# RQLuo/CDLNet-video

Hardware: AMD Instinct MI355X
Metric: Mpix/s denoised (fwd+bwd) at K=30,M=64,P=7 (higher is better)
Workload: dtype f32 (split-bf16 x3 MFMA, fp32 accumulate, fp32 storage)

## Files before the change

### cdlnet-video_amd/csrc/cdl_common.h

```cpp
#pragma once
#include <hip/hip_runtime.h>
#include "../../include/cdlnet_hip.h"

#define CDL_LAUNCH_CHECK()                                   \
    do {                                                     \
        hipError_t e_ = hipGetLastError();                   \
        if (e_ != hipSuccess) return -(int)e_;               \
    } while (0)

__device__ __forceinline__ float cdl_shrink(float u, float t)
{
    float m = fabsf(u) - t;
    m = m > 0.0f ? m : (m != m ? m : 0.0f);
    const float s = u > 0.0f ? 1.0f : (u < 0.0f ? -1.0f : (u != u ? u : 0.0f));
    return s * m;
}

__device__ __forceinline__ float cdl_sgn(float x) { return x > 0.0f ? 1.0f : (x < 0.0f ? -1.0f : 0.0f); }

struct cdl_prox1 {
    float s, ls, a, tg, m, z;
};

__device__ __forceinline__ cdl_prox1 cdl_prox_csr1(float u, float zp, float lam, float gam)
// ... 51 lines not shown

__host__ __device__ __forceinline__ int cdl_floordiv(int a, int b)
{
    int q = a / b;
    return (a % b != 0 && ((a < 0) != (b < 0))) ? q - 1 : q;
}

#ifdef CDL_ABLATE
#define CDL_DBG(flags, bit) (((flags) & (bit)) != 0)
#define CDL_DBG_FIELD(decl) decl
#define CDL_DBG_COMMA(x) , x
#else
#define CDL_DBG(flags, bit) (false)
#define CDL_DBG_FIELD(decl)
#define CDL_DBG_COMMA(x)
#endif

struct cdl_options {
    int mfma_analysis, mfma_synthesis, mfma_wgrad, mfma_dense;
    int no_tiled, no_pipelined_synthesis;
    int fused_snake;
    int fused_grid;
    int fused_da;
    int fusedg_bwd_prec;
    int fusedg_strip;
    int scalar_assemble;
    int fused_debug, dense_debug;
};
const cdl_options &cdl_opts();
bool cdl_exact_fp32();
int cdl_current_device();
int cdl_cu_count();
int cdl_ensure_dynamic_lds(const void *kernel, int bytes);

static inline bool cdl_geom_ok(const cdl_geom *g)
{
    if (!g) return false;
    if (g->N <= 0 || g->C <= 0 || g->M <= 0) return false;
    if (g->D <= 0 || g->H <= 0 || g->W <= 0) return false;
    if (g->Pd <= 0 || g->Ph <= 0 || g->Pw <= 0) return false;
    if (g->sd <= 0 || g->sh <= 0 || g->sw <= 0) return false;
    if (g->pd < 0 || g->ph < 0 || g->pw < 0) return false;
    if (g->D % g->sd || g->H % g->sh || g->W % g->sw) return false;
    return true;
}

// ... 47 lines not shown
```

### cdlnet-video_amd/csrc/cdl_fused2d.hip

```cpp
#include <atomic>
#include <cstdlib>
#include <type_traits>
#include <mutex>
#include <utility>
#include <vector>

#include "cdl_common.h"

#ifdef CDL_F2D_WY4
#define CDL_WY 4
#define cdl_fused2d_assemble cdl_fused2d_assemble_wy4
#define cdl_fused2d_backward cdl_fused2d_backward_wy4
#define cdl_fused2d_code_bytes cdl_fused2d_code_bytes_wy4
#define cdl_fused2d_dtau_reduce cdl_fused2d_dtau_reduce_wy4
#define cdl_fused2d_forward cdl_fused2d_forward_wy4
#define cdl_fused2d_frag_bytes cdl_fused2d_frag_bytes_wy4
#define cdl_fused2d_iter_fwd cdl_fused2d_iter_fwd_wy4
#define cdl_fused2d_map_words cdl_fused2d_map_words_wy4
#define cdl_fused2d_patch_floats cdl_fused2d_patch_floats_wy4
#define cdl_fused2d_prep cdl_fused2d_prep_wy4
#define cdl_fused2d_stage_bwd cdl_fused2d_stage_bwd_wy4
#define cdl_fused2d_support_map cdl_fused2d_support_map_wy4
#define cdl_fused2d_supported cdl_fused2d_supported_wy4
#define cdl_fused2d_tiles cdl_fused2d_tiles_wy4
// ... 21 lines not shown
constexpr int RTW = TW + 2 * HALO, RTH = TH + 2 * HALO;
constexpr int RTC = RTW + 2;
constexpr int PITCH = WY == 2 ? 28 : 44;
constexpr int COPY = RTC * PITCH;
constexpr int LDS_RT = 2 * 4 * COPY * 2;
constexpr int SLAB = RTH * RTW;
constexpr int LDS_RSUM = 4 * SLAB * 4;
constexpr int LDS_W = 32 * 64 * 16;
constexpr int LDS_TAU = 64 * 4;
constexpr int LDS_TACC = NW * 64 * 4;
constexpr int LDS_STAGE = LDS_RT + LDS_RSUM + LDS_W + LDS_TAU + LDS_TACC;

constexpr int GW_TH = 16;
constexpr int GW_RTH = GW_TH + 2 * HALO;
constexpr int TROWS = GW_RTH + 1;
constexpr int TPITCH = 72;
constexpr int TCOPY = TROWS * TPITCH;
constexpr int WG_THIN_BYTES = 2 * 2 * 4 * TCOPY * 2;
constexpr int IMG_ELEMS = 32 * 32;

constexpr int LDS_DA_THIN = 2 * 4 * TCOPY * 2;
constexpr int LDS_DA = LDS_DA_THIN + NW * 2 * 2 * IMG_ELEMS * 2;

struct FusedParams {
    const float *r;
    const float *zin;
    unsigned *map;
    float *zout;
    const float *tau;
    float *dtau;
    const uint4 *frags;
    float *patches;
    float sgn;
    int do_synth;
    CDL_DBG_FIELD(int dbg;)
    int N, H, W, tilesX, tilesY;
    int rev;
    const float *r2;
    float *da_partial;
};

enum { MODE_FWD = 0, MODE_FIRST = 1, MODE_BWD = 2 };

__device__ __forceinline__ float embed7(const float *w, int P, int i, int j)
{
    const int off = (7 - P) / 2;
    const int ii = i - off, jj = j - off;
    if (i > 6 || j > 6 || ii < 0 || jj < 0 || ii >= P || jj >= P) return 0.0f;
    return w[ii * P + jj];
}

__device__ __forceinline__ void prep_one(const float *__restrict__ wA, const float *__restrict__ wB,
                                         uint4 *__restrict__ out, int MT, int P, int t)
{
    const int FA = MT * 4, FB = 4 * MT;
    if (t >= (FA + FB) * 64) return;
    const int lane = t & 63, f = t >> 6;
    const int row = lane & 31, h = lane >> 5;
    const int PP = P * P;
    float v[8];
    if (f < FA) {
        const int R = f / 4, ks = f % 4;
// ... 169 lines not shown
{
    return __builtin_bit_cast(float, __builtin_amdgcn_update_dpp(0, __builtin_bit_cast(int, v), 0x138, 0xf, 0xf, true));
}
__device__ __forceinline__ float upper_half_to_lower(float v)
{
    float lo = 0.0f;
    asm volatile("s_nop 1\n\tv_permlane32_swap_b32 %0, %1\n\ts_nop 1" : "+v"(v), "+v"(lo));
    return lo;
}
__device__ __forceinline__ float col2im_row(const float (&rv)[4], int h)
{
    const float r4 = upper_half_to_lower(rv[0]);
    const float r5 = upper_half_to_lower(rv[1]);
    const float r6 = upper_half_to_lower(rv[2]);
    const bool lo = h == 0;
    float s = lo ? r6 : 0.0f;
    s = wave_shr1(s) + (lo ? r5 : 0.0f);
    s = wave_shr1(s) + (lo ? r4 : 0.0f);
    s = wave_shr1(s) + (lo ? rv[3] : 0.0f);
    s = wave_shr1(s) + (lo ? rv[2] : 0.0f);
    s = wave_shr1(s) + (lo ? rv[1] : 0.0f);
    s = wave_shr1(s) + (lo ? rv[0] : 0.0f);
    return s;
}

template <int MT, int PREC, int MODE, int LIN, int LOUT, bool DA = false>
__global__ __launch_bounds__(NT) void k_stage(FusedParams p)
{
    static_assert(!DA || (MODE == MODE_BWD && TH == GW_TH), "dA_k rides in the reverse stage, on k_wgrad2d's 64 x 16 tiles");
    extern __shared__ __attribute__((aligned(16))) unsigned char smem[];
    __bf16 *rt = reinterpret_cast<__bf16 *>(smem);
    float *rsum_all = reinterpret_cast<float *>(smem + LDS_RT);
    const uint4 *wl = reinterpret_cast<const uint4 *>(smem + LDS_RT + LDS_RSUM);
    float *tau_s = reinterpret_cast<float *>(smem + LDS_RT + LDS_RSUM + LDS_W);
    float *tacc_s = tau_s + 64;
    __bf16 *thin2 = reinterpret_cast<__bf16 *>(smem + LDS_STAGE);
    __bf16 *imgs2 = reinterpret_cast<__bf16 *>(smem + LDS_STAGE + LDS_DA_THIN);

    constexpr int M = 32 * MT;
    constexpr int FA = MT * 4, FB = 4 * MT;
    constexpr int NFRAG = (PREC != 1 ? 2 : 1) * (FA + FB);
    constexpr int NSTG = (RTH * RTW + NT - 1) / NT;
    const int tid = threadIdx.x, lane = tid & 63, wid = tid >> 6;
    const int wxi = wid % WX, wyi = wid / WX;
    const int c = lane & 31, h = lane >> 5;
    const size_t HW = (size_t)p.H * p.W;
// ... 480 lines not shown
    stage_store();
    if constexpr (DA) stage2_store();
    }
    if constexpr (DA) {
        float *red = reinterpret_cast<float *>(smem);
        for (int w = 0; w < NW; ++w) {
            __syncthreads();
            if (wid == w) {
#pragma unroll
                for (int R = 0; R < MT; ++R)
#pragma unroll
                    for (int tt = 0; tt < 2; ++tt)
#pragma unroll
                        for (int v = 0; v < 16; ++v) {
                            const int ch = 32 * R + (v & 3) + 8 * (v >> 2) + 4 * h;
                            float *dstw = &red[ch * 64 + 32 * tt + c];
                            *dstw = (w == 0 ? 0.0f : *dstw) + dacc[R][tt][v];
                        }
            }
        }
        __syncthreads();
        float *dst = p.da_partial + (size_t)blockIdx.x * 2 * M * 64;
        for (int i = tid; i < M * 64; i += NT) dst[i] = red[i];
    }
}

__device__ __forceinline__ float patch_sum(const float *__restrict__ patches, int n, int Y, int X,
                                           int tilesX, int tilesY)
{
    const int tyc = Y / TH, txc = X / TW;
    const int ly = Y - tyc * TH, lx = X - txc * TW;
    const int hx = (lx < HALO && txc > 0) ? -1 : ((lx >= TW - HALO && txc + 1 < tilesX) ? 1 : 0);
    const int vy = (ly < HALO && tyc > 0) ? -1 : ((ly >= TH - HALO && tyc + 1 < tilesY) ? 1 : 0);
    const float *own = patches + (((size_t)n * tilesY + tyc) * tilesX + txc) * SLAB + (ly + HALO) * RTW + lx + HALO;
    const ptrdiff_t dx = (ptrdiff_t)hx * (SLAB - TW), dy = (ptrdiff_t)vy * ((ptrdiff_t)tilesX * SLAB - TH * RTW);
    float sum = 0.0f;
    if (vy < 0) {
        if (hx < 0) sum += own[dy + dx];
        sum += own[dy];
        if (hx > 0) sum += own[dy + dx];
    }
    if (hx < 0) sum += own[dx];
    sum += own[0];
    if (hx > 0) sum += own[dx];
    if (vy > 0) {
        if (hx < 0) sum += own[dy + dx];
// ... 95 lines not shown
    const size_t i = (size_t)blockIdx.x * blockDim.x + threadIdx.x;
    if (i >= (size_t)N * 2 * HW) return;
    const size_t pix = i % HW;
    const int h = (int)((i / HW) % 2), n = (int)(i / (2 * HW));
    unsigned ws = 0, wg = 0;
    for (int R = 0; R < M / 32; ++R)
        for (int v = 0; v < 16; ++v) {
            const int ch = 32 * R + 8 * (v >> 2) + 4 * h + (v & 3);
            const float zz = z[((size_t)n * M + ch) * HW + pix];
            ws |= (zz != 0.0f ? 1u : 0u) << (16 * R + v);
            wg |= (__builtin_bit_cast(unsigned, zz) >> 31) << (16 * R + v);
        }
    map[((size_t)n * 4 + 2 * h) * HW + pix] = ws;
    map[((size_t)n * 4 + 2 * h + 1) * HW + pix] = wg;
}

struct WgradParams {
    const float *X[2];
    const float *T[2];
    float *partial;
    int N, H, W, tilesX, tilesY, numTiles;
    int rev;
    int single;
};

template <int MT, int PREC, int LAY>
__global__ __launch_bounds__(512) void k_wgrad2d(WgradParams p)
{
    extern __shared__ __attribute__((aligned(16))) unsigned char dsm[];
    __bf16 *thin = reinterpret_cast<__bf16 *>(dsm);
    __bf16 *imgs = reinterpret_cast<__bf16 *>(dsm + WG_THIN_BYTES);
    constexpr int M = 32 * MT;
    const int tid = threadIdx.x, lane = tid & 63, wid = tid >> 6;
    const int op = wid >> 2, wq = wid & 3;
    const int wxi = wq & 1, wyi = wq >> 1;
    const int c = lane & 31, h = lane >> 5;
    const size_t HW = (size_t)p.H * p.W;
    __bf16 *wimg = imgs + (size_t)wid * (MT * 2) * IMG_ELEMS;
    f32x16 acc[MT][2];
#pragma unroll
    for (int R = 0; R < MT; ++R)
#pragma unroll
        for (int tt = 0; tt < 2; ++tt)
#pragma unroll
            for (int v = 0; v < 16; ++v) acc[R][tt][v] = 0.0f;

    for (int i = tid; i < WG_THIN_BYTES / 16; i += 512) reinterpret_cast<uint4 *>(dsm)[i] = make_uint4(0, 0, 0, 0);

    const bool present = p.X[op] != nullptr;
    const int nsteps = p.single ? (p.numTiles + 1) / 2 : p.numTiles;
    for (int t0 = blockIdx.x; t0 < nsteps; t0 += gridDim.x) {
        const int t = p.single ? 2 * t0 + op : t0;
        const bool active = present && t < p.numTiles;
        int bid = p.rev ? p.numTiles - 1 - t : t;
        const int txi = bid % p.tilesX; bid /= p.tilesX;
        const int tyi = bid % p.tilesY;
        const int n = active ? bid / p.tilesY : 0;
        const int tx0 = txi * TW, ty0 = tyi * GW_TH;
        __syncthreads();
        if (active) {
            const float *timg = p.T[op] + (size_t)n * HW;
            constexpr int NSW = (GW_RTH * RTW + 255) / 256;
            float tv[NSW];
#pragma unroll
            for (int k = 0; k < NSW; ++k) {
                const int i = (tid & 255) + k * 256;
                const int yy = i / RTW, xx = i % RTW;
                const int gy = ty0 - HALO + yy, gx = tx0 - HALO + xx;
                const bool ok = i < GW_RTH * RTW && gy >= 0 && gy < p.H && gx >= 0 && gx < p.W;
                const float v = timg[ok ? (size_t)gy * p.W + gx : 0];
                tv[k] = ok ? v : 0.0f;
            }
#pragma unroll
            for (int k = 0; k < NSW; ++k) {
                const int i = (tid & 255) + k * 256;
                if (i >= GW_RTH * RTW) continue;
                const int yy = i / RTW, xx = i % RTW;
                const __bf16 hh = (__bf16)tv[k];
                const __bf16 ll = (__bf16)(tv[k] - (float)hh);
#pragma unroll
                for (int s = 0; s < 4; ++s)
                    if (xx - s >= 0) {
                        thin[((op * 2 + 0) * 4 + s) * TCOPY + yy * TPITCH + xx - s] = hh;
                        if (PREC != 1) thin[((op * 2 + 1) * 4 + s) * TCOPY + yy * TPITCH + xx - s] = ll;
                    }
            }
        }
        __syncthreads();
        if (!active) continue;

        const int x = tx0 + wxi * 32 + c;
        const bool xok = x < p.W;
#pragma unroll 1
        for (int b = 0; b < RB; ++b) {
// ... 92 lines not shown
            __builtin_amdgcn_wave_barrier();
        }
    }

    float *red = reinterpret_cast<float *>(dsm);
    for (int w = 0; w < 4; ++w) {
        __syncthreads();
        if (wq == w) {
#pragma unroll
            for (int R = 0; R < MT; ++R)
#pragma unroll
                for (int tt = 0; tt < 2; ++tt)
#pragma unroll
                    for (int v = 0; v < 16; ++v) {
                        const int ch = 32 * R + (v & 3) + 8 * (v >> 2) + 4 * h;
                        float *dstw = &red[(op * M + ch) * 64 + 32 * tt + c];
                        *dstw = (w == 0 ? 0.0f : *dstw) + acc[R][tt][v];
                    }
        }
    }
    __syncthreads();
    float *dst = p.partial + (size_t)blockIdx.x * 2 * M * 64;
    for (int i = tid; i < 2 * M * 64; i += 512) dst[i] = red[i];
}

__global__ __launch_bounds__(1024) void k_wgrad_reduce(const float *__restrict__ partial, int G,
                                                       float *__restrict__ dw0, float alpha0,
                                                       float *__restrict__ dw1, float alpha1, int M, int P, int merge = 0)
{
    __shared__ float red[32][33];
    const int o = threadIdx.x & 31, part = threadIdx.x >> 5;
    const int t = blockIdx.x * 32 + o;
    const int per = M * P * P;
    const bool live = t < (merge ? per : 2 * per);
    float sum = 0.0f;
    int op = 0, r = 0;
    if (live) {
        op = t / per; r = t % per;
        const int ch = r / (P * P), ij = r % (P * P), off = (7 - P) / 2;
        const int tap = 8 * (ij / P + off) + (ij % P + off);
        for (int g = part; g < G; g += 32) {
            sum += partial[((size_t)(g * 2 + op) * M + ch) * 64 + tap];
            if (merge) sum += partial[((size_t)(g * 2 + 1) * M + ch) * 64 + tap];
        }
    }
    red[part][o] = sum;
// ... 14 lines not shown
                                                      float *__restrict__ dt1, int N, int per_img, int M)
{
    __shared__ float r0[256][4], r1[256][4];
    const int mi = threadIdx.x & 3, part = threadIdx.x >> 2;
    const int m = blockIdx.x * 4 + mi;
    float a0 = 0.0f, a1 = 0.0f;
    const int rows = N * per_img;
    if (m < M)
        for (int row = part; row < rows; row += 256) {
            const float v = partial[(size_t)row * M + m];
            a0 += v;
            if (c) a1 = fmaf(c[row / per_img], v, a1);
        }
    r0[part][mi] = a0;
    r1[part][mi] = a1;
    __syncthreads();
    for (int stride = 128; stride >= 1; stride >>= 1) {
        if (part < stride) { r0[part][mi] += r0[part + stride][mi]; r1[part][mi] += r1[part + stride][mi]; }
        __syncthreads();
    }
    if (part == 0 && m < M) { dt0[m] = r0[0][mi]; dt1[m] = r1[0][mi]; }
}

inline hipStream_t S(void *s) { return reinterpret_cast<hipStream_t>(s); }

inline bool fused_shape_ok(const cdl_geom *g)
{
    if (!cdl_geom_ok(g)) return false;
    if (g->C != 1 || g->D != 1 || g->Pd != 1 || g->sd != 1 || g->sh != 1 || g->sw != 1) return false;
    if (g->Ph != g->Pw || g->Ph > 7 || (g->Ph & 1) == 0 || g->ph != g->Ph / 2 || g->pw != g->Pw / 2) return false;
    if (g->M != 32 && g->M != 64) return false;
    if (blk_image_elems(g->M, g->H, g->W) * 4 >= ((size_t)1 << 31)) return false;
    return true;
}

inline int debug_flags() { return cdl_opts().fused_debug; }

inline int tiles_x(const cdl_geom *g) { return (g->W + TW - 1) / TW; }
inline int tiles_y(const cdl_geom *g) { return (g->H + TH - 1) / TH; }

struct Flags {
    int prec, rev, lin, lout;
    bool ok;
};
inline Flags parse_flags(int precision)
{
// ... 32 lines not shown
    CDL_LAY_CASE(LAY_NCHW, LAY_NCHW);
    CDL_LAY_CASE(LAY_BLK, LAY_BLK);
    CDL_LAY_CASE(LAY_BLK16, LAY_BLK16);
    if constexpr (MODE == MODE_FWD) {
        CDL_LAY_CASE(LAY_BLK, LAY_NCHW);
        CDL_LAY_CASE(LAY_BLK16, LAY_NCHW);
    }
    if constexpr (MODE == MODE_BWD) {
        CDL_LAY_CASE(LAY_NCHW, LAY_BLK);
        CDL_LAY_CASE(LAY_NCHW, LAY_BLK16);
    }
#undef CDL_LAY_CASE
    return CDL_EUNSUPPORTED;
}

template <int MT, int PREC>
int launch_stage(const FusedParams &p, int mode, int lin, int lout, dim3 grid, hipStream_t st)
{
    if (mode == MODE_FWD) return launch_stage_lay<MT, PREC, MODE_FWD>(p, lin, lout, grid, st);
    if (mode == MODE_FIRST) return launch_stage_lay<MT, PREC, MODE_FIRST>(p, lin, lout, grid, st);
    return launch_stage_lay<MT, PREC, MODE_BWD>(p, lin, lout, grid, st);
}

int stage_grid(const cdl_geom *, const FusedParams &p)
{
    const size_t tiles = (size_t)p.N * p.tilesX * p.tilesY;
    size_t cus = (size_t)cdl_cu_count();
    const int cap = cdl_opts().fused_grid;
    if (cap > 0 && (size_t)cap < cus) cus = (size_t)cap;
    return (int)(tiles < cus ? tiles : cus);
}

int dispatch_stage(const cdl_geom *g, const FusedParams &p, int mode, const Flags &f, hipStream_t st)
{
    dim3 grid((unsigned)stage_grid(g, p));
    if (g->M == 64)
        return f.prec == 0   ? launch_stage<2, 0>(p, mode, f.lin, f.lout, grid, st)
               : f.prec == 1 ? launch_stage<2, 1>(p, mode, f.lin, f.lout, grid, st)
                             : launch_stage<2, 2>(p, mode, f.lin, f.lout, grid, st);
    return f.prec == 0   ? launch_stage<1, 0>(p, mode, f.lin, f.lout, grid, st)
           : f.prec == 1 ? launch_stage<1, 1>(p, mode, f.lin, f.lout, grid, st)
                         : launch_stage<1, 2>(p, mode, f.lin, f.lout, grid, st);
}

int wgrad_grid(const cdl_geom *g)
{
    const size_t tiles = (size_t)g->N * tiles_x(g) * ((g->H + GW_TH - 1) / GW_TH);
    return (int)(tiles < 512 ? tiles : 512);
}

template <int MT, int PREC, int LAY>
int launch_wgrad_one(const WgradParams &p, int G, hipStream_t st)
{
    const size_t lds = (size_t)WG_THIN_BYTES + (size_t)8 * MT * 2 * IMG_ELEMS * 2;
    if (int rc = cdl_ensure_dynamic_lds((const void *)k_wgrad2d<MT, PREC, LAY>, (int)lds)) return rc;
    k_wgrad2d<MT, PREC, LAY><<<G, 512, lds, st>>>(p);
    hipError_t e = hipGetLastError();
    return e == hipSuccess ? 0 : -(int)e;
}

template <int MT, int PREC>
int launch_wgrad(const WgradParams &p, int lay, int G, hipStream_t st)
{
    if (lay == LAY_BLK) return launch_wgrad_one<MT, PREC, LAY_BLK>(p, G, st);
    if (lay == LAY_BLK16) return launch_wgrad_one<MT, PREC, LAY_BLK16>(p, G, st);
    return launch_wgrad_one<MT, PREC, LAY_NCHW>(p, G, st);
}

}

extern "C" {

int cdl_fused2d_supported(const cdl_geom *g) { return fused_shape_ok(g) ? 1 : 0; }

size_t cdl_fused2d_frag_bytes(int M) { return (size_t)2 * (M / 32) * 8 * 64 * 16; }

#ifndef CDL_F2D_WY4
size_t cdl_fused2d_patch_floats_wy4(const cdl_geom *g);
size_t cdl_fused2d_tiles_wy4(const cdl_geom *g);
size_t cdl_fused2d_wgrad_workspace_floats_wy4(const cdl_geom *g);
static size_t larger(size_t a, size_t b) { return a > b ? a : b; }
#else
static size_t larger(size_t a, size_t) { return a; }
#endif

size_t cdl_fused2d_patch_floats(const cdl_geom *g)
{
    if (!fused_shape_ok(g)) return 0;
    const size_t own = (size_t)g->N * tiles_x(g) * tiles_y(g) * SLAB;
#ifndef CDL_F2D_WY4
// ... 48 lines not shown
    return 0;
}

int cdl_fused2d_iter_fwd(const cdl_geom *g, const float *r, const float *zin, const float *tau,
                         const void *frags, float sgn, float *zout, float *patches, unsigned *map_out,
                         int precision, void *stream)
{
    if (!fused_shape_ok(g)) return CDL_EUNSUPPORTED;
    if (!r || !tau || !frags || !zout || !patches || zout == zin) return CDL_EINVAL;
    const Flags f = parse_flags(precision);
    if (!f.ok) return CDL_EINVAL;
    FusedParams p = {};
    p.rev = f.rev;
    p.r = r; p.zin = zin; p.zout = zout; p.tau = tau; p.map = map_out;
    p.frags = reinterpret_cast<const uint4 *>(frags);
    p.patches = patches; p.sgn = sgn; p.do_synth = 1; CDL_DBG_FIELD(p.dbg = debug_flags();)
    p.N = g->N; p.H = g->H; p.W = g->W;
    p.tilesX = tiles_x(g); p.tilesY = tiles_y(g);
    return dispatch_stage(g, p, zin ? MODE_FWD : MODE_FIRST, f, S(stream));
}

static int stage_bwd(const cdl_geom *g, const float *thin, const float *base, const unsigned *map, const void *frags,
                     float *du_out, float *patches, float *dtau_partial, int do_synth, int precision, const float *r2,
                     float alpha, float *dA, float *workspace, void *stream)
{
    if (!fused_shape_ok(g)) return CDL_EUNSUPPORTED;
    if (!thin || !map || !frags || !du_out || !dtau_partial || du_out == base) return CDL_EINVAL;
    if (do_synth && !patches) return CDL_EINVAL;
    if (r2 && (!dA || !workspace)) return CDL_EINVAL;
    const Flags f = parse_flags(precision);
    if (!f.ok) return CDL_EINVAL;
    FusedParams p = {};
    p.rev = f.rev;
    p.r = thin; p.zin = base; p.map = const_cast<unsigned *>(map); p.zout = du_out; p.dtau = dtau_partial;
    p.frags = reinterpret_cast<const uint4 *>(frags);
    p.patches = patches; p.sgn = 1.0f; p.do_synth = do_synth ? 1 : 0; CDL_DBG_FIELD(p.dbg = debug_flags();)
    p.N = g->N; p.H = g->H; p.W = g->W;
    p.tilesX = tiles_x(g); p.tilesY = tiles_y(g);
    p.r2 = r2; p.da_partial = workspace;
    int rc = dispatch_stage(g, p, MODE_BWD, f, S(stream));
    if (rc || !r2) return rc;
    const int G = stage_grid(g, p);
    const int total = 2 * g->M * g->Ph * g->Pw;
    k_wgrad_reduce<<<(total + 31) / 32, 1024, 0, S(stream)>>>(workspace, G, dA, alpha, nullptr, 0.0f, g->M, g->Ph);
    CDL_LAUNCH_CHECK();
    return 0;
}

int cdl_fused2d_stage_bwd(const cdl_geom *g, const float *thin, const float *base, const unsigned *map,
                          const void *frags, float *du_out, float *patches, float *dtau_partial, int do_synth,
                          const float *r2, float alpha, float *dA, float *workspace, int precision, void *stream)
{
    if (!r2 != !dA || !r2 != !workspace) return CDL_EINVAL;
    return stage_bwd(g, thin, base, map, frags, du_out, patches, dtau_partial, do_synth, precision, r2, alpha, dA, workspace,
                     stream);
}

int cdl_fused2d_dtau_reduce(const cdl_geom *g, const float *dtau_partial, const float *c, float *dt0, float *dt1,
                            float *dtau_n, void *stream)
{
    if (!fused_shape_ok(g)) return CDL_EUNSUPPORTED;
    if (!dtau_partial || !dt0 || !dt1) return CDL_EINVAL;
    const int per_img = tiles_x(g) * tiles_y(g);
    k_dtau_reduce<<<(g->M + 3) / 4, 1024, 0, S(stream)>>>(dtau_partial, c, dt0, dt1, g->N, per_img, g->M);
    CDL_LAUNCH_CHECK();
    if (!dtau_n) return 0;
    return cdl_dtau_per_sample(dtau_partial, g->N, g->M, per_img, (size_t)per_img * g->M, 1, g->M, dtau_n, stream);
}

size_t cdl_fused2d_wgrad_workspace_floats(const cdl_geom *g)
{
    if (!fused_shape_ok(g)) return 0;
    const size_t own = (size_t)wgrad_grid(g) * 2 * g->M * 64;
#ifndef CDL_F2D_WY4
    return larger(own, cdl_fused2d_wgrad_workspace_floats_wy4(g));
#else
    return own;
#endif
}

int cdl_fused2d_wgrad(const cdl_geom *g, const float *X0, const float *T0, float alpha0, float *dw0,
                      const float *X1, const float *T1, float alpha1, float *dw1, float *workspace,
                      int precision, void *stream)
{
    if (!fused_shape_ok(g)) return CDL_EUNSUPPORTED;
    if (!workspace || (!X0 && !X1)) return CDL_EINVAL;
    if ((X0 && (!T0 || !dw0)) || (X1 && (!T1 || !dw1))) return CDL_EINVAL;
    const Flags f = parse_flags(precision);
    if (!f.ok) return CDL_EINVAL;
    WgradParams p = {};
    p.rev = f.rev;
    p.X[0] = X0; p.T[0] = T0; p.X[1] = X1; p.T[1] = T1;
    p.single = (X0 != nullptr) != (X1 != nullptr);
    if (p.single) {
        if (!X0) { X0 = X1; T0 = T1; alpha0 = alpha1; dw0 = dw1; X1 = nullptr; }
        p.X[0] = p.X[1] = X0; p.T[0] = p.T[1] = T0;
    }
    p.partial = workspace;
    p.N = g->N; p.H = g->H; p.W = g->W;
    p.tilesX = tiles_x(g); p.tilesY = (g->H + GW_TH - 1) / GW_TH;
    p.numTiles = p.N * p.tilesX * p.tilesY;
    int G = wgrad_grid(g);
    if (p.single && G > (p.numTiles + 1) / 2) G = (p.numTiles + 1) / 2;
    int rc;
    if (g->M == 64)
        rc = f.prec == 0 ? launch_wgrad<2, 0>(p, f.lin, G, S(stream))
             : f.prec == 1 ? launch_wgrad<2, 1>(p, f.lin, G, S(stream)) : launch_wgrad<2, 2>(p, f.lin, G, S(stream));
    else
        rc = f.prec == 0 ? launch_wgrad<1, 0>(p, f.lin, G, S(stream))
             : f.prec == 1 ? launch_wgrad<1, 1>(p, f.lin, G, S(stream)) : launch_wgrad<1, 2>(p, f.lin, G, S(stream));
    if (rc) return rc;
    const int total = 2 * g->M * g->Ph * g->Pw;
    k_wgrad_reduce<<<(total + 31) / 32, 1024, 0, S(stream)>>>(workspace, G, X0 ? dw0 : nullptr, alpha0,
                                                             X1 ? dw1 : nullptr, alpha1, g->M, g->Ph, p.single);
    CDL_LAUNCH_CHECK();
    return 0;
}

int cdl_fused2d_assemble(const cdl_geom *g, const float *patches, const float *mask, const float *sub,
                         float alpha, float *out, float *acc, int acc_add, void *stream)
{
    if (!fused_shape_ok(g)) return CDL_EUNSUPPORTED;
    if (!patches || (!out && !acc)) return CDL_EINVAL;
    if ((size_t)g->N * g->H * g->W >= ((size_t)1 << 20) && (g->W & 3) == 0 && !cdl_opts().scalar_assemble) {
        dim3 grid((unsigned)((g->W + 255) / 256), (unsigned)((g->H + 7) / 8), (unsigned)g->N);
        k_assemble_v4<<<grid, 256, 0, S(stream)>>>(patches, mask, sub, alpha, out, g->N, g->H, g->W, tiles_x(g), tiles_y(g), acc, acc_add);
    } else if ((size_t)g->N * g->H * g->W >= ((size_t)1 << 20)) {
        dim3 grid((unsigned)((g->W + 255) / 256), (unsigned)((g->H + 3) / 4), (unsigned)g->N);
        k_assemble<4><<<grid, 256, 0, S(stream)>>>(patches, mask, sub, alpha, out, g->N, g->H, g->W, tiles_x(g), tiles_y(g), acc, acc_add);
    } else {
        dim3 grid((unsigned)((g->W + 255) / 256), (unsigned)g->H, (unsigned)g->N);
        k_assemble<1><<<grid, 256, 0, S(stream)>>>(patches, mask, sub, alpha, out, g->N, g->H, g->W, tiles_x(g), tiles_y(g), acc, acc_add);
    }
    CDL_LAUNCH_CHECK();
// ... 143 lines not shown
    if (rc) return rc;
    for (int k = 0; k < K; ++k) {
        const void *fk = static_cast<const char *>(frags) + (size_t)k * fb;
        {
            TimingScope ts(k ? 0 : 3, S(stream));
            rc = cdl_fused2d_iter_fwd(g, thin, k ? z[k - 1] : nullptr, tau + k * nm, fk, k ? -1.0f : 1.0f, z[k],
                                      patches, maps ? maps[k] : nullptr,
                                      f.prec | CDL_LAYOUT_IN(L) | CDL_LAYOUT_OUT(k == K - 1 ? LAY_NCHW : L) |
                                          ((k & 1) && snake ? CDL_TILES_REVERSED : 0),
                                      stream);
        }
        if (rc) return rc;
        if (k < K - 1) {
            rc = cdl_fused2d_assemble(g, patches, mask, yp, 1.0f, r[k], nullptr, 0, stream);
            thin = r[k];
        } else {
            rc = cdl_fused2d_assemble(g, patches, nullptr, nullptr, 1.0f, xp, nullptr, 0, stream);
        }
        if (rc) return rc;
    }
    return 0;
}

int cdl_fused2d_backward(const cdl_geom *g, int K, const float *yp, const float *mask, const float *c,
                         const float *const *wA, const float *const *wB, const float *const *z,
                         const float *const *r, const unsigned *const *maps, const float *g_xp,
                         const float *g_z, float *const *dA,
                         float *const *dB, float *dt, float *du0, float *du1, float *q, void *frags,
                         float *patches, float *dtau_partial, float *wgrad_ws, int precision, float *dyp,
                         float *dtau, void *stream)
{
    if (!fused_shape_ok(g)) return CDL_EUNSUPPORTED;
    if (K < 1 || !yp || !wA || !wB || !z || !maps || !g_xp || !dA || !dB || !dt || !du0 || !du1 || !q || !frags ||
        !patches || !dtau_partial || !wgrad_ws || (K > 1 && !r))
        return CDL_EINVAL;
    const int M = g->M;
    float *du[2] = {du0, du1};
    const Flags f = parse_flags(precision);
    if (!f.ok || f.lout != 0) return CDL_EINVAL;
    const int L = f.lin;
#ifndef CDL_F2D_WY4
    if (L == LAY_BLK16)
        return cdl_fused2d_backward_wy4(g, K, yp, mask, c, wA, wB, z, r, maps, g_xp, g_z, dA, dB, dt, du0, du1, q, frags,
                                        patches, dtau_partial, wgrad_ws, precision, dyp, dtau, stream);
#endif
    const int sdir = snake_enabled() ? (((K - 1) & 1) ? CDL_TILES_REVERSED : 0) : 0;
    const int wdir = snake_enabled() ? (sdir ^ CDL_TILES_REVERSED) : 0;
    const int sprec = f.prec | sdir, wprec = f.prec | wdir;
    int rc = cdl_fused2d_wgrad(g, z[K - 1], g_xp, 1.0f, dB[0], nullptr, nullptr, 0.0f, nullptr, wgrad_ws,
                               wprec, stream);
    if (rc) return rc;
    const float *thin = g_xp, *base = g_z;
    const size_t fb = cdl_fused2d_frag_bytes(M);
    rc = prep_pairs(wB, wA, K, 0, frags, M, g->Ph, S(stream));
    if (rc) return rc;
    for (int k = K - 1, flip = 0; k >= 0; --k, flip ^= 1) {
        const void *fk = static_cast<const char *>(frags) + (size_t)k * fb;
        float *duk = du[flip];
        const bool ride = TH == GW_TH && cdl_opts().fused_da;
        {
            TimingScope ts(1, S(stream));
            rc = stage_bwd(g, thin, base, maps[k], fk, duk, patches, dtau_partial, k >= 1 || dyp,
                           sprec | CDL_LAYOUT_IN(k == K - 1 ? LAY_NCHW : L) | CDL_LAYOUT_OUT(L),
                           ride ? (k >= 1 ? r[k - 1] : yp) : nullptr, k >= 1 ? -1.0f : 1.0f, dA[k], wgrad_ws, stream);
        }
        if (rc) return rc;
        rc = cdl_fused2d_dtau_reduce(g, dtau_partial, c, dt + (size_t)k * 2 * M, dt + (size_t)k * 2 * M + M,
                                     dtau ? dtau + (size_t)k * g->N * M : nullptr, stream);
        if (rc) return rc;
        if (k == 0 && dyp) {
            rc = cdl_fused2d_assemble(g, patches, nullptr, nullptr, 1.0f, nullptr, dyp, K > 1, stream);
            if (rc) return rc;
        }
        if (k >= 1) {
            rc = cdl_fused2d_assemble(g, patches, mask, nullptr, -1.0f, q, dyp, k < K - 1, stream);
            if (rc) return rc;
            {
                TimingScope ts(2, S(stream));
                rc = ride ? cdl_fused2d_wgrad(g, z[k - 1], q, 1.0f, dB[k], nullptr, nullptr, 0.0f, nullptr, wgrad_ws,
                                              wprec | CDL_LAYOUT_IN(L), stream)
                          : cdl_fused2d_wgrad(g, duk, r[k - 1], -1.0f, dA[k], z[k - 1], q, 1.0f, dB[k], wgrad_ws,
                                              wprec | CDL_LAYOUT_IN(L), stream);
// ... 14 lines not shown
```

### cdlnet-video_amd/csrc/cdl_options.hip

```cpp
#include <atomic>
#include <cstdlib>
#include <map>
#include <mutex>
#include <utility>

#include "cdl_common.h"

namespace {

std::atomic<const cdl_options *> g_opts{nullptr};
std::mutex g_opts_mutex;

int env_int(const char *name, int dflt)
{
    const char *e = getenv(name);
    return (e && *e) ? atoi(e) : dflt;
}
int env_flag_off(const char *name)
{
    const char *e = getenv(name);
    return (e && e[0] == '0') ? 0 : 1;
}

const cdl_options *load_options()
{
    cdl_options *o = new cdl_options;
    o->mfma_analysis = env_flag_off("CDL_MFMA_ANALYSIS");
    o->mfma_synthesis = env_flag_off("CDL_MFMA_SYNTHESIS");
    o->mfma_wgrad = env_flag_off("CDL_MFMA_WGRAD");
    o->mfma_dense = env_flag_off("CDL_MFMA_DENSE");
    o->no_tiled = getenv("CDL_NO_TILED") ? 1 : 0;
    o->no_pipelined_synthesis = getenv("CDL_NO_PIPELINED_SYNTHESIS") ? 1 : 0;
    o->fused_snake = env_flag_off("CDL_FUSED_SNAKE");
    o->fused_grid = env_int("CDL_FUSED_GRID", 0);
    o->fused_da = env_flag_off("CDL_FUSED_DA");
    o->scalar_assemble = env_int("CDL_SCALAR_ASSEMBLE", 0) ? 1 : 0;
    o->fusedg_strip = env_int("CDL_FUSEDG_STRIP", 0) ? 1 : 0;
    o->fusedg_bwd_prec = env_int("CDL_FUSEDG_PREC", -1);
#ifdef CDL_ABLATE
    o->fused_debug = env_int("CDL_FUSED_DEBUG", 0);
    o->dense_debug = env_int("CDL_DENSE_DEBUG", 0);
#else
    o->fused_debug = o->dense_debug = 0;
#endif
    return o;
}

thread_local int t_exact_fp32 = 0;

constexpr int MAX_DEV = 64;
std::atomic<int> g_cus[MAX_DEV];
std::mutex g_attr_mutex;
std::map<std::pair<int, const void *>, int> g_attr_bytes;

}

const cdl_options &cdl_opts()
{
// ... 59 lines not shown
```

Before: 115.6.

## Fold wgrad/dtau reductions and patch assembly into neighbouring backward kernels

Adds a folded backward path, on by default through CDL_FUSED_FOLD. The previous stage's weight-gradient reduction now runs in the tail of the next stage kernel, and dA and dtau reductions run in the tail of the wgrad kernel. The wgrad kernel also assembles overlapping patch sums into q and dyp directly, replacing the separate assemble launch. This removes several small kernel launches and extra global round trips per unrolled iteration. In exchange the tail reductions are serialised per workgroup and need a larger workspace.

```diff
diff --git a/cdlnet-video_amd/csrc/cdl_common.h b/cdlnet-video_amd/csrc/cdl_common.h
--- a/cdlnet-video_amd/csrc/cdl_common.h
+++ b/cdlnet-video_amd/csrc/cdl_common.h
@@ -97,6 +97,7 @@
     int fused_snake;
     int fused_grid;
     int fused_da;
+    int fused_fold;
     int fusedg_bwd_prec;
     int fusedg_strip;
     int scalar_assemble;
diff --git a/cdlnet-video_amd/csrc/cdl_fused2d.hip b/cdlnet-video_amd/csrc/cdl_fused2d.hip
--- a/cdlnet-video_amd/csrc/cdl_fused2d.hip
+++ b/cdlnet-video_amd/csrc/cdl_fused2d.hip
@@ -67,6 +67,18 @@
 constexpr int LDS_DA_THIN = 2 * 4 * TCOPY * 2;
 constexpr int LDS_DA = LDS_DA_THIN + NW * 2 * 2 * IMG_ELEMS * 2;
 
+struct WgradRed {
+    const float *partial;
+    float *dw;
+    float alpha;
+    int G, merge, M, P;
+};
+struct DtauRed {
+    const float *partial;
+    const float *c;
+    float *dt0, *dt1, *dtau_n;
+    int N, per_img, M;
+};
 struct FusedParams {
     const float *r;
     const float *zin;
@@ -83,6 +95,7 @@
     int rev;
     const float *r2;
     float *da_partial;
+    WgradRed dB;
 };
 
 enum { MODE_FWD = 0, MODE_FIRST = 1, MODE_BWD = 2 };
@@ -298,6 +311,99 @@
     s = wave_shr1(s) + (lo ? rv[1] : 0.0f);
     s = wave_shr1(s) + (lo ? rv[0] : 0.0f);
     return s;
+}
+
+constexpr int RED_CH = 64;
+constexpr int RED_B = 16;
+
+__device__ void wgrad_reduce_slice(const WgradRed &r, float *lds, int tid, int nt)
+{
+    const int PP = r.P * r.P, per = r.M * PP, off = (7 - r.P) / 2;
+    const int S = (per + (int)gridDim.x - 1) / (int)gridDim.x;
+    const int o0 = (int)blockIdx.x * S, o1 = min(per, o0 + S);
+    for (int b = o0; b < o1; b += RED_CH) {
+        const int n = min(RED_CH, o1 - b);
+        for (int i = tid; i < 32 * n; i += nt) {
+            const int part = i / n, j = i - part * n;
+            const int rr = b + j, ch = rr / PP, ij = rr - ch * PP;
+            const int tap = 8 * (ij / r.P + off) + (ij % r.P + off);
+            float sum = 0.0f;
+            for (int g0 = part; g0 < r.G; g0 += 32 * RED_B) {
+                float v0[RED_B], v1[RED_B];
+#pragma unroll
+                for (int u = 0; u < RED_B; ++u) {
+                    const int g = g0 + 32 * u < r.G ? g0 + 32 * u : 0;
+                    v0[u] = r.partial[((size_t)(g * 2) * r.M + ch) * 64 + tap];
+                    v1[u] = r.partial[((size_t)(g * 2 + 1) * r.M + ch) * 64 + tap];
+                }
+#pragma unroll
+                for (int u = 0; u < RED_B; ++u)
+                    if (g0 + 32 * u < r.G) {
+                        sum += v0[u];
+                        if (r.merge) sum += v1[u];
+                    }
+            }
+            lds[part * RED_CH + j] = sum;
+        }
+        __syncthreads();
+        if (tid < n) {
+            float tot = 0.0f;
+            for (int k = 0; k < 32; ++k) tot += lds[k * RED_CH + tid];
+            r.dw[b + tid] = r.alpha * tot;
+        }
+        __syncthreads();
+    }
+}
+
+__device__ void dtau_reduce_slice(const DtauRed &d, float *lds, int tid, int nt)
+{
+    const int grp = tid >> 8, part = tid & 255, ngrp = nt >> 8;
+    float *r0 = lds + grp * 512, *r1 = r0 + 256;
+    const int rows = d.N * d.per_img;
+    for (int mb = (int)blockIdx.x * ngrp; mb < d.M; mb += (int)gridDim.x * ngrp) {
+        const int m = mb + grp;
+        float a0 = 0.0f, a1 = 0.0f;
+        if (m < d.M)
+            for (int row0 = part; row0 < rows; row0 += 256 * RED_B) {
+                float v[RED_B], cv[RED_B];
+#pragma unroll
+                for (int u = 0; u < RED_B; ++u) {
+                    const int row = row0 + 256 * u < rows ? row0 + 256 * u : 0;
+                    v[u] = d.partial[(size_t)row * d.M + m];
+                    cv[u] = d.c ? d.c[row / d.per_img] : 0.0f;
+                }
+#pragma unroll
+                for (int u = 0; u < RED_B; ++u)
+                    if (row0 + 256 * u < rows) {
+                        a0 += v[u];
+                        if (d.c) a1 = fmaf(cv[u], v[u], a1);
+                    }
+            }
+        r0[part] = a0;
+        r1[part] = a1;
+        __syncthreads();
+        for (int stride = 128; stride >= 1; stride >>= 1) {
+            if (part < stride) { r0[part] += r0[part + stride]; r1[part] += r1[part + stride]; }
+            __syncthreads();
+        }
+        if (part == 0 && m < d.M) { d.dt0[m] = r0[0]; d.dt1[m] = r1[0]; }
+        __syncthreads();
+    }
+    if (d.dtau_n)
+        for (int i = (int)blockIdx.x + (int)gridDim.x * tid; i < d.N * d.M; i += (int)gridDim.x * nt) {
+            const int n = i / d.M, m = i - n * d.M;
+            const float *pp = d.partial + (size_t)n * d.per_img * d.M + m;
+            float a = 0.0f;
+            for (int j0 = 0; j0 < d.per_img; j0 += RED_B) {
+                float v[RED_B];
+#pragma unroll
+                for (int u = 0; u < RED_B; ++u) v[u] = pp[(size_t)(j0 + u < d.per_img ? j0 + u : 0) * d.M];
+#pragma unroll
+                for (int u = 0; u < RED_B; ++u)
+                    if (j0 + u < d.per_img) a += v[u];
+            }
+            d.dtau_n[i] = a;
+        }
 }
 
 template <int MT, int PREC, int MODE, int LIN, int LOUT, bool DA = false>
@@ -824,6 +930,7 @@
         __syncthreads();
         float *dst = p.da_partial + (size_t)blockIdx.x * 2 * M * 64;
         for (int i = tid; i < M * 64; i += NT) dst[i] = red[i];
+        if (p.dB.dw) wgrad_reduce_slice(p.dB, reinterpret_cast<float *>(thin2), tid, NT);
     }
 }
 
@@ -965,6 +1072,13 @@
     int N, H, W, tilesX, tilesY, numTiles;
     int rev;
     int single;
+    const float *patches;
+    const float *qmask;
+    float qalpha;
+    float *qout, *dyp;
+    int dyp_add;
+    WgradRed dA;
+    DtauRed dtau;
 };
 
 template <int MT, int PREC, int LAY>
@@ -1002,17 +1116,66 @@
         const int tx0 = txi * TW, ty0 = tyi * GW_TH;
         __syncthreads();
         if (active) {
-            const float *timg = p.T[op] + (size_t)n * HW;
             constexpr int NSW = (GW_RTH * RTW + 255) / 256;
             float tv[NSW];
-#pragma unroll
-            for (int k = 0; k < NSW; ++k) {
-                const int i = (tid & 255) + k * 256;
-                const int yy = i / RTW, xx = i % RTW;
-                const int gy = ty0 - HALO + yy, gx = tx0 - HALO + xx;
-                const bool ok = i < GW_RTH * RTW && gy >= 0 && gy < p.H && gx >= 0 && gx < p.W;
-                const float v = timg[ok ? (size_t)gy * p.W + gx : 0];
-                tv[k] = ok ? v : 0.0f;
+            if (p.patches) {
+                const size_t pimg = (size_t)p.tilesY * p.tilesX * SLAB;
+                const __amdgpu_buffer_rsrc_t rp = uniform_rsrc(p.patches + (size_t)n * pimg, pimg * 4);
+                const __amdgpu_buffer_rsrc_t rm = uniform_rsrc(p.qmask ? p.qmask + (size_t)n * HW : p.patches, p.qmask ? HW * 4 : 0);
+                auto nbr = [&](int i, int &gy, int &gx, int &hx, int &vy, int &own) __attribute__((always_inline)) {
+                    const int yy = i / RTW, xx = i % RTW;
+                    gy = ty0 - HALO + yy; gx = tx0 - HALO + xx;
+                    const bool ok = i < GW_RTH * RTW && gy >= 0 && gy < p.H && gx >= 0 && gx < p.W;
+                    const int Y = ok ? gy : 0, X = ok ? gx : 0;
+                    const int tyc = Y / TH, txc = X / TW, ly0 = Y - tyc * TH, lx0 = X - txc * TW;
+                    hx = !ok ? 2 : (lx0 < HALO && txc > 0) ? -1 : ((lx0 >= TW - HALO && txc + 1 < p.tilesX) ? 1 : 0);
+                    vy = (ly0 < HALO && tyc > 0) ? -1 : ((ly0 >= TH - HALO && tyc + 1 < p.tilesY) ? 1 : 0);
+                    own = (tyc * p.tilesX + txc) * SLAB + (ly0 + HALO) * RTW + lx0 + HALO;
+                };
+                float l0[NSW], lx[NSW], ly[NSW], lxy[NSW], mk[NSW];
+#pragma unroll
+                for (int k = 0; k < NSW; ++k) {
+                    int gy, gx, hx, vy, own;
+                    nbr((tid & 255) + k * 256, gy, gx, hx, vy, own);
+                    const int dx = (hx & 1) ? hx * (SLAB - TW) : 0, dy = vy * (p.tilesX * SLAB - TH * RTW);
+                    const bool ok = hx != 2, hn = (hx & 1) != 0, vn = vy != 0;
+                    l0[k] = buf_ld(rp, ok ? own * 4 : OOB, 0);
+                    lx[k] = buf_ld(rp, hn ? (own + dx) * 4 : OOB, 0);
+                    ly[k] = buf_ld(rp, vn ? (own + dy) * 4 : OOB, 0);
+                    lxy[k] = buf_ld(rp, hn && vn ? (own + dy + dx) * 4 : OOB, 0);
+                    mk[k] = buf_ld(rm, ok ? (gy * p.W + gx) * 4 : OOB, 0);
+                }
+#pragma unroll
+                for (int k = 0; k < NSW; ++k) {
+                    int gy, gx, hx, vy, own;
+                    nbr((tid & 255) + k * 256, gy, gx, hx, vy, own);
+                    float s = 0.0f;
+                    if (vy < 0) { if (hx < 0) s += lxy[k]; s += ly[k]; if (hx == 1) s += lxy[k]; }
+                    if (hx < 0) s += lx[k];
+                    s += l0[k];
+                    if (hx == 1) s += lx[k];
+                    if (vy > 0) { if (hx < 0) s += lxy[k]; s += ly[k]; if (hx == 1) s += lxy[k]; }
+                    float v = p.qalpha * s;
+                    if (p.qmask) v *= mk[k];
+                    tv[k] = hx == 2 ? 0.0f : v;
+                    const int yy = gy - (ty0 - HALO), xx = gx - (tx0 - HALO);
+                    if (hx != 2 && yy >= HALO && yy < HALO + GW_TH && xx >= HALO && xx < HALO + TW) {
+                        const size_t gi = (size_t)n * HW + (size_t)gy * p.W + gx;
+                        p.qout[gi] = v;
+                        if (p.dyp) p.dyp[gi] = p.dyp_add ? p.dyp[gi] + s : s;
+                    }
+                }
+            } else {
+                const float *timg = p.T[op] + (size_t)n * HW;
+#pragma unroll
+                for (int k = 0; k < NSW; ++k) {
+                    const int i = (tid & 255) + k * 256;
+                    const int yy = i / RTW, xx = i % RTW;
+                    const int gy = ty0 - HALO + yy, gx = tx0 - HALO + xx;
+                    const bool ok = i < GW_RTH * RTW && gy >= 0 && gy < p.H && gx >= 0 && gx < p.W;
+                    const float v = timg[ok ? (size_t)gy * p.W + gx : 0];
+                    tv[k] = ok ? v : 0.0f;
+                }
             }
 #pragma unroll
             for (int k = 0; k < NSW; ++k) {
@@ -1151,6 +1314,9 @@
     __syncthreads();
     float *dst = p.partial + (size_t)blockIdx.x * 2 * M * 64;
     for (int i = tid; i < 2 * M * 64; i += 512) dst[i] = red[i];
+    float *scr = reinterpret_cast<float *>(dsm + WG_THIN_BYTES);
+    if (p.dA.dw) wgrad_reduce_slice(p.dA, scr, tid, 512);
+    if (p.dtau.partial) dtau_reduce_slice(p.dtau, scr, tid, 512);
 }
 
 __global__ __launch_bounds__(1024) void k_wgrad_reduce(const float *__restrict__ partial, int G,
@@ -1211,6 +1377,27 @@
     if (part == 0 && m < M) { dt0[m] = r0[0][mi]; dt1[m] = r1[0][mi]; }
 }
 
+struct TailParams {
+    WgradRed dA;
+    DtauRed dtau;
+    const float *patches;
+    float *dyp;
+    int dyp_add, N, H, W, tilesX, tilesY;
+};
+__global__ __launch_bounds__(256) void k_rev_tail(TailParams p)
+{
+    __shared__ float lds[32 * RED_CH];
+    if (p.dA.dw) wgrad_reduce_slice(p.dA, lds, threadIdx.x, 256);
+    if (p.dtau.partial) dtau_reduce_slice(p.dtau, lds, threadIdx.x, 256);
+    if (!p.dyp) return;
+    const size_t total = (size_t)p.N * p.H * p.W;
+    for (size_t i = (size_t)blockIdx.x * 256 + threadIdx.x; i < total; i += (size_t)gridDim.x * 256) {
+        const int X = (int)(i % p.W), Y = (int)((i / p.W) % p.H), n = (int)(i / ((size_t)p.W * p.H));
+        const float raw = patch_sum(p.patches, n, Y, X, p.tilesX, p.tilesY);
+        p.dyp[i] = p.dyp_add ? p.dyp[i] + raw : raw;
+    }
+}
+
 inline hipStream_t S(void *s) { return reinterpret_cast<hipStream_t>(s); }
 
 inline bool fused_shape_ok(const cdl_geom *g)
@@ -1289,9 +1476,9 @@
     return launch_stage_lay<MT, PREC, MODE_BWD>(p, lin, lout, grid, st);
 }
 
-int stage_grid(const cdl_geom *, const FusedParams &p)
-{
-    const size_t tiles = (size_t)p.N * p.tilesX * p.tilesY;
+int stage_grid(const cdl_geom *g)
+{
+    const size_t tiles = (size_t)g->N * tiles_x(g) * tiles_y(g);
     size_t cus = (size_t)cdl_cu_count();
     const int cap = cdl_opts().fused_grid;
     if (cap > 0 && (size_t)cap < cus) cus = (size_t)cap;
@@ -1300,7 +1487,7 @@
 
 int dispatch_stage(const cdl_geom *g, const FusedParams &p, int mode, const Flags &f, hipStream_t st)
 {
-    dim3 grid((unsigned)stage_grid(g, p));
+    dim3 grid((unsigned)stage_grid(g));
     if (g->M == 64)
         return f.prec == 0   ? launch_stage<2, 0>(p, mode, f.lin, f.lout, grid, st)
                : f.prec == 1 ? launch_stage<2, 1>(p, mode, f.lin, f.lout, grid, st)
@@ -1333,6 +1520,23 @@
     if (lay == LAY_BLK16) return launch_wgrad_one<MT, PREC, LAY_BLK16>(p, G, st);
     return launch_wgrad_one<MT, PREC, LAY_NCHW>(p, G, st);
 }
+
+int wgrad_partials(const cdl_geom *g, WgradParams &p, const Flags &f, hipStream_t st, int *G)
+{
+    p.rev = f.rev;
+    p.N = g->N; p.H = g->H; p.W = g->W;
+    p.tilesX = tiles_x(g); p.tilesY = (g->H + GW_TH - 1) / GW_TH;
+    p.numTiles = p.N * p.tilesX * p.tilesY;
+    *G = wgrad_grid(g);
+    if (p.single && *G > (p.numTiles + 1) / 2) *G = (p.numTiles + 1) / 2;
+    if (g->M == 64)
+        return f.prec == 0 ? launch_wgrad<2, 0>(p, f.lin, *G, st)
+               : f.prec == 1 ? launch_wgrad<2, 1>(p, f.lin, *G, st) : launch_wgrad<2, 2>(p, f.lin, *G, st);
+    return f.prec == 0 ? launch_wgrad<1, 0>(p, f.lin, *G, st)
+           : f.prec == 1 ? launch_wgrad<1, 1>(p, f.lin, *G, st) : launch_wgrad<1, 2>(p, f.lin, *G, st);
+}
+
+size_t wgrad_bank_floats(const cdl_geom *g) { return (size_t)wgrad_grid(g) * 2 * g->M * 64; }
 
 }
 
@@ -1427,12 +1631,13 @@
 
 static int stage_bwd(const cdl_geom *g, const float *thin, const float *base, const unsigned *map, const void *frags,
                      float *du_out, float *patches, float *dtau_partial, int do_synth, int precision, const float *r2,
-                     float alpha, float *dA, float *workspace, void *stream)
+                     float alpha, float *dA, float *workspace, void *stream, const WgradRed *fold_dB = nullptr)
 {
     if (!fused_shape_ok(g)) return CDL_EUNSUPPORTED;
     if (!thin || !map || !frags || !du_out || !dtau_partial || du_out == base) return CDL_EINVAL;
     if (do_synth && !patches) return CDL_EINVAL;
     if (r2 && (!dA || !workspace)) return CDL_EINVAL;
+    if (fold_dB && !r2) return CDL_EINVAL;
     const Flags f = parse_flags(precision);
     if (!f.ok) return CDL_EINVAL;
     FusedParams p = {};
@@ -1443,9 +1648,10 @@
     p.N = g->N; p.H = g->H; p.W = g->W;
     p.tilesX = tiles_x(g); p.tilesY = tiles_y(g);
     p.r2 = r2; p.da_partial = workspace;
+    if (fold_dB) p.dB = *fold_dB;
     int rc = dispatch_stage(g, p, MODE_BWD, f, S(stream));
-    if (rc || !r2) return rc;
-    const int G = stage_grid(g, p);
+    if (rc || !r2 || fold_dB) return rc;
+    const int G = stage_grid(g);
     const int total = 2 * g->M * g->Ph * g->Pw;
     k_wgrad_reduce<<<(total + 31) / 32, 1024, 0, S(stream)>>>(workspace, G, dA, alpha, nullptr, 0.0f, g->M, g->Ph);
     CDL_LAUNCH_CHECK();
@@ -1476,7 +1682,8 @@
 size_t cdl_fused2d_wgrad_workspace_floats(const cdl_geom *g)
 {
     if (!fused_shape_ok(g)) return 0;
-    const size_t own = (size_t)wgrad_grid(g) * 2 * g->M * 64;
+    const size_t tiles = (size_t)g->N * tiles_x(g) * tiles_y(g), cus = (size_t)cdl_cu_count();
+    const size_t own = wgrad_bank_floats(g) + (TH == GW_TH ? (tiles < cus ? tiles : cus) * 2 * g->M * 64 : 0);
 #ifndef CDL_F2D_WY4
     return larger(own, cdl_fused2d_wgrad_workspace_floats_wy4(g));
 #else
@@ -1494,7 +1701,6 @@
     const Flags f = parse_flags(precision);
     if (!f.ok) return CDL_EINVAL;
     WgradParams p = {};
-    p.rev = f.rev;
     p.X[0] = X0; p.T[0] = T0; p.X[1] = X1; p.T[1] = T1;
     p.single = (X0 != nullptr) != (X1 != nullptr);
     if (p.single) {
@@ -1502,19 +1708,8 @@
         p.X[0] = p.X[1] = X0; p.T[0] = p.T[1] = T0;
     }
     p.partial = workspace;
-    p.N = g->N; p.H = g->H; p.W = g->W;
-    p.tilesX = tiles_x(g); p.tilesY = (g->H + GW_TH - 1) / GW_TH;
-    p.numTiles = p.N * p.tilesX * p.tilesY;
-    int G = wgrad_grid(g);
-    if (p.single && G > (p.numTiles + 1) / 2) G = (p.numTiles + 1) / 2;
-    int rc;
-    if (g->M == 64)
-        rc = f.prec == 0 ? launch_wgrad<2, 0>(p, f.lin, G, S(stream))
-             : f.prec == 1 ? launch_wgrad<2, 1>(p, f.lin, G, S(stream)) : launch_wgrad<2, 2>(p, f.lin, G, S(stream));
-    else
-        rc = f.prec == 0 ? launch_wgrad<1, 0>(p, f.lin, G, S(stream))
-             : f.prec == 1 ? launch_wgrad<1, 1>(p, f.lin, G, S(stream)) : launch_wgrad<1, 2>(p, f.lin, G, S(stream));
-    if (rc) return rc;
+    int G = 0;
+    if (int rc = wgrad_partials(g, p, f, S(stream), &G)) return rc;
     const int total = 2 * g->M * g->Ph * g->Pw;
     k_wgrad_reduce<<<(total + 31) / 32, 1024, 0, S(stream)>>>(workspace, G, X0 ? dw0 : nullptr, alpha0,
                                                              X1 ? dw1 : nullptr, alpha1, g->M, g->Ph, p.single);
@@ -1704,6 +1899,65 @@
     return 0;
 }
 
+static int backward_folded(const cdl_geom *g, int K, const float *yp, const float *mask, const float *c,
+                           const float *const *wA, const float *const *wB, const float *const *z, const float *const *r,
+                           const unsigned *const *maps, const float *g_xp, const float *g_z, float *const *dA,
+                           float *const *dB, float *dt, float *const *du, float *q, void *frags, float *patches,
+                           float *dtau_partial, float *wgrad_ws, int L, int sprec, int wprec, float *dyp, float *dtau,
+                           hipStream_t st)
+{
+    const int M = g->M, P = g->Ph;
+    float *const wsW = wgrad_ws, *const wsA = wgrad_ws + wgrad_bank_floats(g);
+    const int Gs = stage_grid(g), per_img = tiles_x(g) * tiles_y(g);
+    int Gw = 0, rc;
+    {
+        WgradParams p = {};
+        p.X[0] = p.X[1] = z[K - 1]; p.T[0] = p.T[1] = g_xp; p.single = 1; p.partial = wsW;
+        if ((rc = wgrad_partials(g, p, parse_flags(wprec), st, &Gw))) return rc;
+    }
+    WgradRed pend = {wsW, dB[0], 1.0f, Gw, 1, M, P};
+    const size_t fb = cdl_fused2d_frag_bytes(M);
+    if ((rc = prep_pairs(wB, wA, K, 0, frags, M, P, st))) return rc;
+    const float *thin = g_xp, *base = g_z;
+    for (int k = K - 1, flip = 0; k >= 0; --k, flip ^= 1) {
+        const void *fk = static_cast<const char *>(frags) + (size_t)k * fb;
+        float *duk = du[flip];
+        {
+            TimingScope ts(1, st);
+            rc = stage_bwd(g, thin, base, maps[k], fk, duk, patches, dtau_partial, k >= 1 || dyp,
+                           sprec | CDL_LAYOUT_IN(k == K - 1 ? LAY_NCHW : L) | CDL_LAYOUT_OUT(L), k >= 1 ? r[k - 1] : yp,
+                           k >= 1 ? -1.0f : 1.0f, dA[k], wsA, st, &pend);
+        }
+        if (rc) return rc;
+        const WgradRed redA = {wsA, dA[k], k >= 1 ? -1.0f : 1.0f, Gs, 0, M, P};
+        const DtauRed redT = {dtau_partial, c, dt + (size_t)k * 2 * M, dt + (size_t)k * 2 * M + M,
+                              dtau ? dtau + (size_t)k * g->N * M : nullptr, g->N, per_img, M};
+        if (k >= 1) {
+            TimingScope ts(2, st);
+            WgradParams p = {};
+            p.X[0] = p.X[1] = z[k - 1]; p.single = 1; p.partial = wsW;
+            p.patches = patches; p.qmask = mask; p.qalpha = -1.0f; p.qout = q; p.dyp = dyp; p.dyp_add = k < K - 1;
+            p.dA = redA; p.dtau = redT;
+            rc = wgrad_partials(g, p, parse_flags(wprec | CDL_LAYOUT_IN(L)), st, &Gw);
+            pend = {wsW, dB[k], 1.0f, Gw, 1, M, P};
+            thin = q;
+        } else {
+            TailParams tp = {};
+            tp.dA = redA; tp.dtau = redT;
+            tp.patches = patches; tp.dyp = dyp; tp.dyp_add = K > 1;
+            tp.N = g->N; tp.H = g->H; tp.W = g->W; tp.tilesX = tiles_x(g); tp.tilesY = tiles_y(g);
+            const size_t pix = (size_t)g->N * g->H * g->W;
+            const size_t wgs = dyp ? (pix + 1023) / 1024 : (size_t)Gs;
+            k_rev_tail<<<(unsigned)(wgs < 65535 ? wgs : 65535), 256, 0, st>>>(tp);
+            hipError_t e = hipGetLastError();
+            rc = e == hipSuccess ? 0 : -(int)e;
+        }
+        if (rc) return rc;
+        base = duk;
+    }
+    return 0;
+}
+
 int cdl_fused2d_backward(const cdl_geom *g, int K, const float *yp, const float *mask, const float *c,
                          const float *const *wA, const float *const *wB, const float *const *z,
                          const float *const *r, const unsigned *const *maps, const float *g_xp,
@@ -1729,6 +1983,10 @@
     const int sdir = snake_enabled() ? (((K - 1) & 1) ? CDL_TILES_REVERSED : 0) : 0;
     const int wdir = snake_enabled() ? (sdir ^ CDL_TILES_REVERSED) : 0;
     const int sprec = f.prec | sdir, wprec = f.prec | wdir;
+    const bool ride = TH == GW_TH && cdl_opts().fused_da;
+    if (ride && cdl_opts().fused_fold)
+        return backward_folded(g, K, yp, mask, c, wA, wB, z, r, maps, g_xp, g_z, dA, dB, dt, du, q, frags, patches,
+                               dtau_partial, wgrad_ws, L, sprec, wprec, dyp, dtau, S(stream));
     int rc = cdl_fused2d_wgrad(g, z[K - 1], g_xp, 1.0f, dB[0], nullptr, nullptr, 0.0f, nullptr, wgrad_ws,
                                wprec, stream);
     if (rc) return rc;
@@ -1739,7 +1997,6 @@
     for (int k = K - 1, flip = 0; k >= 0; --k, flip ^= 1) {
         const void *fk = static_cast<const char *>(frags) + (size_t)k * fb;
         float *duk = du[flip];
-        const bool ride = TH == GW_TH && cdl_opts().fused_da;
         {
             TimingScope ts(1, S(stream));
             rc = stage_bwd(g, thin, base, maps[k], fk, duk, patches, dtau_partial, k >= 1 || dyp,
diff --git a/cdlnet-video_amd/csrc/cdl_options.hip b/cdlnet-video_amd/csrc/cdl_options.hip
--- a/cdlnet-video_amd/csrc/cdl_options.hip
+++ b/cdlnet-video_amd/csrc/cdl_options.hip
@@ -34,6 +34,7 @@
     o->fused_snake = env_flag_off("CDL_FUSED_SNAKE");
     o->fused_grid = env_int("CDL_FUSED_GRID", 0);
     o->fused_da = env_flag_off("CDL_FUSED_DA");
+    o->fused_fold = env_flag_off("CDL_FUSED_FOLD");
     o->scalar_assemble = env_int("CDL_SCALAR_ASSEMBLE", 0) ? 1 : 0;
     o->fusedg_strip = env_int("CDL_FUSEDG_STRIP", 0) ? 1 : 0;
     o->fusedg_bwd_prec = env_int("CDL_FUSEDG_PREC", -1);
```

Result: no change. 116.0, median of 6 (+0.4%).
